# equinor/gordo-components

Hardware: NVIDIA H100
Metric: anomaly windows/sec (64-tag feedforward_hourglass AE, 1k machines x 10k rows per GPU, fused predict+score) (higher is better)
Workload: dtype split tf32/bf16/fp16

## Files before the change

gordo_components_b200/csrc/ffae_infer_tc.cu:

```cuda
#include <atomic>
#include <cuda_bf16.h>
#include <cuda_fp16.h>
#include "gb_common.cuh"
#include "gb_sm90.cuh"

namespace {

using namespace gb::sm90;

constexpr int TILE = 64;
constexpr int NWG_MAX = 3;
constexpr int MAXL = 8;
constexpr int W = 64;
constexpr int BOX_COLS = 32;
constexpr int BOX_COLS_X64 = 16;
constexpr int BOX_BYTES = TILE * BOX_COLS * 4;
constexpr int TILE_BYTES = 2 * BOX_BYTES;
__host__ __device__ constexpr int x_tile_bytes(bool x64) { return x64 ? 2 * TILE_BYTES : TILE_BYTES; }
__host__ __device__ constexpr int stage_bytes(bool x64, int nwg) { return (x_tile_bytes(x64) + TILE_BYTES) * nwg; }
constexpr int OBOX_ROWS = 16;
constexpr int OBOX_BYTES = OBOX_ROWS * BOX_COLS * 4;
__host__ __device__ constexpr int restage_batch(int nthreads) { return (W * W + W + nthreads - 1) / nthreads; }
static_assert(restage_batch(128 * NWG_MAX) == 11, "three warpgroups restage a layer in 11 loads per thread");

struct TcArgs {
  CUtensorMap tm_x, tm_y;
  CUtensorMap tm_o[4];
  int T;
  int L;
  int N[MAXL], Np[MAXL], k16[MAXL];
  int img0_ofs[MAXL], img1_ofs[MAXL], img2_ofs[MAXL];
  int bias_ofs[MAXL];
  int pofs[MAXL];
  int K[MAXL];
  int w_bytes;
  int vec_ofs;
  int stage_ofs;
  int n_jobs, tiles_per_job;
  long pstride;
  const float* params;
  const gb_job* jobs;
  const float *y, *scale, *feat_thr, *agg_thr;
  float *o_model, *o_ts, *o_tu, *o_conf, *o_tots, *o_totu, *o_totconf;
  unsigned int* work_ctr;
  const double *x_scale, *x_offset;
  int xab_ofs;
  long n_x_rows;
};

constexpr float TANH_ARG_SCALE = 2.8853900817779268f;
__device__ __forceinline__ float tanh_from_scaled(float t) {
  float e, r;
  asm("ex2.approx.ftz.f32 %0, %1;" : "=f"(e) : "f"(t));
  asm("rcp.approx.ftz.f32 %0, %1;" : "=f"(r) : "f"(e + 1.0f));
// ... 22 lines not shown
#pragma unroll
  for (int ks = 0; ks < 8; ++ks)
    if (ks < 2 * k16) {
      const uint32_t a[4] = {xhi[ks >> 1][4 * (ks & 1) + 0], xhi[ks >> 1][4 * (ks & 1) + 1], xhi[ks >> 1][4 * (ks & 1) + 2], xhi[ks >> 1][4 * (ks & 1) + 3]};
      if (N == 16) wgmma_rs_tf32_n16(d, a, desc_noswizzle(img0 + ks * step, lbo, 128), ks > 0);
      if (N == 32) wgmma_rs_tf32_n32(d, a, desc_noswizzle(img0 + ks * step, lbo, 128), ks > 0);
      if (N == 48) wgmma_rs_tf32_n48(d, a, desc_noswizzle(img0 + ks * step, lbo, 128), ks > 0);
      if (N == 64) wgmma_rs_tf32_n64(d, a, desc_noswizzle(img0 + ks * step, lbo, 128), ks > 0);
    }
#pragma unroll
  for (int ks = 0; ks < 4; ++ks)
    if (ks < k16) {
      if (N == 16) wgmma_rs_bf16_n16(d, alo[ks], desc_noswizzle(img1 + ks * step, lbo, 128), 1);
      if (N == 32) wgmma_rs_bf16_n32(d, alo[ks], desc_noswizzle(img1 + ks * step, lbo, 128), 1);
      if (N == 48) wgmma_rs_bf16_n48(d, alo[ks], desc_noswizzle(img1 + ks * step, lbo, 128), 1);
      if (N == 64) wgmma_rs_bf16_n64(d, alo[ks], desc_noswizzle(img1 + ks * step, lbo, 128), 1);
    }
#pragma unroll
  for (int ks = 0; ks < 4; ++ks)
    if (ks < k16) {
      if (N == 16) wgmma_rs_bf16_n16(d, abf[ks], desc_noswizzle(img2 + ks * step, lbo, 128), 1);
      if (N == 32) wgmma_rs_bf16_n32(d, abf[ks], desc_noswizzle(img2 + ks * step, lbo, 128), 1);
      if (N == 48) wgmma_rs_bf16_n48(d, abf[ks], desc_noswizzle(img2 + ks * step, lbo, 128), 1);
      if (N == 64) wgmma_rs_bf16_n64(d, abf[ks], desc_noswizzle(img2 + ks * step, lbo, 128), 1);
    }
}
template <int N>
__device__ __forceinline__ void mma_f16(float* d, const uint32_t* a, uint64_t desc, uint32_t acc) {
  if (N == 16) wgmma_rs_f16_n16(d, a, desc, acc);
  if (N == 32) wgmma_rs_f16_n32(d, a, desc, acc);
  if (N == 48) wgmma_rs_f16_n48(d, a, desc, acc);
  if (N == 64) wgmma_rs_f16_n64(d, a, desc, acc);
}
template <int N>
__device__ __forceinline__ void mma_hidden(float* d, const uint32_t (&a1)[4][4], const uint32_t (&a2)[4][4], uint32_t img0, uint32_t img1, int k16) {
  const uint32_t lbo = N * 16, step = 2 * N * 16;
#pragma unroll
  for (int ks = 0; ks < 4; ++ks)
    if (ks < k16) mma_f16<N>(d, a2[ks], desc_noswizzle(img0 + ks * step, lbo, 128), ks > 0);
#pragma unroll
  for (int ks = 0; ks < 4; ++ks)
    if (ks < k16) mma_f16<N>(d, a1[ks], desc_noswizzle(img1 + ks * step, lbo, 128), 1);
#pragma unroll
  for (int ks = 0; ks < 4; ++ks)
    if (ks < k16) mma_f16<N>(d, a1[ks], desc_noswizzle(img0 + ks * step, lbo, 128), 1);
}

__device__ __forceinline__ int box_ofs(int r, int col) { return r * 128 + (((col >> 2) ^ (r & 7)) << 4) + ((col & 3) << 2); }
__device__ __forceinline__ int tile_ofs(int r, int col) { return (col >> 5) * BOX_BYTES + box_ofs(r, col & 31); }
__device__ __forceinline__ int tile_ofs_x64(int r, int col) { return (col >> 4) * BOX_BYTES + r * 128 + ((((col & 15) >> 1) ^ (r & 7)) << 4); }

__device__ __forceinline__ void warpgroup_sync(int wg) { asm volatile("bar.sync %0, 128;" ::"r"(wg + 1) : "memory"); }

__device__ __forceinline__ void fence_acc(float (&d)[32]) {
#pragma unroll
  for (int i = 0; i < 32; ++i) fence_reg(d[i]);
}
template <int R, int C>
__device__ __forceinline__ void fence_frag(uint32_t (&f)[R][C]) {
#pragma unroll
  for (int i = 0; i < R; ++i)
#pragma unroll
    for (int j = 0; j < C; ++j) fence_reg(f[i][j]);
}

template <bool X64, int NWG>
__global__ void __launch_bounds__(128 * NWG, 1) ffae_tc_kernel(const __grid_constant__ TcArgs a) {
  constexpr int NTHREADS = 128 * NWG;
  constexpr int RESTAGE_BATCH = restage_batch(NTHREADS);
  extern __shared__ __align__(1024) uint8_t smem[];
  const int tid = threadIdx.x, lane = tid & 31;
  const int warp = __shfl_sync(0xffffffffu, tid >> 5, 0);
  const int wg = warp >> 2, wq = warp & 3;
  const int g = lane >> 2, t = lane & 3;
  const uint32_t sbase = smem_u32(smem);
  const int TP = a.T, L = a.L;
  const bool has_y = a.y != nullptr;
  const bool totals = has_y && (a.o_tots || a.o_totu || a.o_totconf);
  const float inv_w = 1.0f / (float)TP;

  __shared__ __align__(8) unsigned long long s_bar[2 * NWG];
  const uint32_t stage = (sbase + a.stage_ofs + 1023) & ~1023u;
  const uint32_t xbuf = stage + wg * (x_tile_bytes(X64) + TILE_BYTES), ybuf = xbuf + x_tile_bytes(X64);
  const uint8_t* xs = smem + (xbuf - sbase);
  const uint8_t* ys = smem + (ybuf - sbase);
  const uint32_t bar_x = smem_u32(&s_bar[wg]), bar_y = smem_u32(&s_bar[NWG + wg]);
  const bool leader = (tid & 127) == 0;
  uint32_t x_phase = 0, y_phase = 0;
  const uint32_t obox0 = ybuf + wq * OBOX_BYTES, obox1 = obox0 + BOX_BYTES;
  if (tid == 0) {
    for (int i = 0; i < 2 * NWG; ++i) mbar_init(smem_u32(&s_bar[i]), 1);
    asm volatile("fence.mbarrier_init.release.cluster;" ::: "memory");
  }

  __shared__ int s_item[3];
  __shared__ int s_range[2];
  if (tid == 0) s_range[0] = s_range[1] = 0;
  int cur_slot = -1;

  while (true) {
    if (tid == 0) {
      const int tpj = a.tiles_per_job, g_total = a.n_jobs * tpj;
      int gg = s_range[0], g_end = s_range[1];
      if (gg >= g_end) {
        const int seen = (int)*reinterpret_cast<volatile unsigned int*>(a.work_ctr);
        const int left = g_total - seen, per_cta = left / (int)gridDim.x;
        int size = per_cta * 2 >= 3 * tpj ? tpj : (per_cta >= tpj / 3 ? (tpj + 2) / 3 : (tpj + 5) / 6);
        if (size < 1) size = 1;
        if (seen % tpj != 0 && size > tpj - seen % tpj) size = tpj - seen % tpj;
        gg = (int)atomicAdd(a.work_ctr, (unsigned int)size);
        g_end = gg + size < g_total ? gg + size : g_total;
      }
      if (gg >= g_total) {
        s_item[0] = -1;
      } else {
        const int job_id = gg / tpj, tile_begin = gg - job_id * tpj;
        const int tile_end = min(tpj, tile_begin + (g_end - gg));
        s_item[0] = job_id; s_item[1] = tile_begin; s_item[2] = tile_end;
        gg += tile_end - tile_begin;
      }
      s_range[0] = gg; s_range[1] = g_end;
    }
    __syncthreads();
    const int job_id = s_item[0], tile_begin = s_item[1], tile_end = s_item[2];
    if (job_id < 0) break;
    const gb_job job = a.jobs[job_id];
    const int row_begin = tile_begin * TILE;
    if (row_begin >= job.n_rows) {
      __syncthreads();
      continue;
    }
    const int row_end = min(job.n_rows, tile_end * TILE);
    const int n_tiles = (row_end - row_begin + TILE - 1) / TILE;

    auto load_tile = [&](const CUtensorMap* m, uint32_t buf, uint32_t bar, int tt) {
      const int row = (int)(job.x_row + row_begin + tt * TILE);
      mbar_expect_tx(bar, TILE_BYTES);
      tma_load_2d(buf, m, 0, row, bar);
      tma_load_2d(buf + BOX_BYTES, m, BOX_COLS, row, bar);
    };
    auto load_x64 = [&](int tt) {
      const int row = (int)(job.x_row + row_begin + tt * TILE);
      mbar_expect_tx(bar_x, x_tile_bytes(true));
#pragma unroll
      for (int h = 0; h < 4; ++h) tma_load_2d(xbuf + h * BOX_BYTES, &a.tm_x, BOX_COLS_X64 * h, row, bar_x);
    };
    if (leader && wg < n_tiles) {
      if constexpr (X64) load_x64(wg);
      else load_tile(&a.tm_x, xbuf, bar_x, wg);
    }

    if (job.slot != cur_slot) {
      cur_slot = job.slot;
      const float* P = a.params + (long)job.slot * a.pstride;
      float v[RESTAGE_BATCH], vn[RESTAGE_BATCH];
      auto fetch = [&](float (&dst)[RESTAGE_BATCH], int l) {
        const float* Ws = P + a.pofs[l];
        const int n_l = a.K[l] * a.N[l] + a.N[l];
#pragma unroll
        for (int u = 0; u < RESTAGE_BATCH; ++u) {
          const int i = tid + u * NTHREADS;
          dst[u] = i < n_l ? __ldg(Ws + i) : 0.f;
        }
      };
      fetch(v, 0);
      const bool vt = tid < TP;
      const float sc = vt && a.scale ? __ldg(a.scale + (long)job.slot * TP + tid) : 0.f;
      const float ft = vt && a.feat_thr ? __ldg(a.feat_thr + (long)job.slot * TP + tid) : 0.f;
      for (int i = tid; i < a.w_bytes / 16; i += NTHREADS) reinterpret_cast<uint4*>(smem)[i] = make_uint4(0, 0, 0, 0);
      __syncthreads();
      for (int l = 0; l < L; ++l) {
        if (l + 1 < L) fetch(vn, l + 1);
        const int K = a.K[l], N = a.N[l], Np = a.Np[l], KN = K * N;
        const float bscale = (l + 1 < L) ? TANH_ARG_SCALE : 1.0f;
#pragma unroll
        for (int u = 0; u < RESTAGE_BATCH; ++u) {
          const int i = tid + u * NTHREADS;
          if (i >= KN + N) break;
          if (i >= KN) {
            reinterpret_cast<float*>(smem + a.bias_ofs[l])[i - KN] = v[u] * bscale;
            continue;
          }
          const int k = i / N, n = i - k * N;
          const float w = v[u];
          const int i8 = ((k >> 3) * Np + n) * 8 + (k & 7);
          if (l == 0) {
            const float hi = __uint_as_float((__float_as_uint(w) + 0x1000u) & 0xffffe000u);
            const int kt = tf32_row(k);
            reinterpret_cast<float*>(smem + a.img0_ofs[0])[((kt >> 2) * Np + n) * 4 + (kt & 3)] = hi;
            reinterpret_cast<__nv_bfloat16*>(smem + a.img1_ofs[0])[i8] = __float2bfloat16_rn(hi);
            reinterpret_cast<__nv_bfloat16*>(smem + a.img2_ofs[0])[i8] = __float2bfloat16_rn(w - hi);
          } else {
            const __half w1 = __float2half_rn(w);
            reinterpret_cast<__half*>(smem + a.img0_ofs[l])[i8] = w1;
            reinterpret_cast<__half*>(smem + a.img1_ofs[l])[i8] = __float2half_rn(w - __half2float(w1));
          }
        }
#pragma unroll
        for (int u = 0; u < RESTAGE_BATCH; ++u) v[u] = vn[u];
      }
      float* vec = reinterpret_cast<float*>(smem + a.vec_ofs);
      if (tid < W) {
        vec[tid] = sc;
        vec[W + tid] = vt && a.feat_thr ? 1.0f / ft : 0.f;
      }
      if constexpr (X64) {
        double* xab = reinterpret_cast<double*>(smem + a.xab_ofs);
        if (tid < W) {
          xab[tid] = vt ? __ldg(a.x_scale + (long)job.slot * TP + tid) : 0.0;
          xab[W + tid] = vt ? __ldg(a.x_offset + (long)job.slot * TP + tid) : 0.0;
        }
      }
      fence_proxy_async();
    }
    __syncthreads();

    const float* vec = reinterpret_cast<const float*>(smem + a.vec_ofs);
    for (int tt = wg; tt < n_tiles; tt += NWG) {
      float d[32];
      uint32_t a1[4][4] = {}, a2[4][4] = {};
      {
        float xr[2][16];
        mbar_wait(bar_x, x_phase);
        x_phase ^= 1;
        if constexpr (X64) {
          const double* xab = reinterpret_cast<const double*>(smem + a.xab_ofs);
          const long row0 = job.x_row + row_begin + tt * TILE + wq * 16 + g;
#pragma unroll
          for (int hr = 0; hr < 2; ++hr) {
            const bool live = row0 + 8 * hr < a.n_x_rows;
#pragma unroll
            for (int c = 0; c < 8; ++c) {
              const int col = 8 * c + 2 * t;
              const double2 v = *reinterpret_cast<const double2*>(xs + tile_ofs_x64(wq * 16 + g + 8 * hr, col));
              const double2 s = *reinterpret_cast<const double2*>(xab + col), o = *reinterpret_cast<const double2*>(xab + W + col);
              xr[hr][2 * c] = live ? (float)__dadd_rn(__dmul_rn(v.x, s.x), o.x) : 0.f;
              xr[hr][2 * c + 1] = live ? (float)__dadd_rn(__dmul_rn(v.y, s.y), o.y) : 0.f;
            }
          }
        } else {
#pragma unroll
          for (int hr = 0; hr < 2; ++hr)
#pragma unroll
            for (int c = 0; c < 8; ++c) {
              const float2 v = *reinterpret_cast<const float2*>(xs + tile_ofs(wq * 16 + g + 8 * hr, 8 * c + 2 * t));
              xr[hr][2 * c] = v.x;
              xr[hr][2 * c + 1] = v.y;
            }
        }
        if (lane == 0) bulk_wait_read<0>();
        warpgroup_sync(wg);
        if (leader) {
          if (tt + NWG < n_tiles) {
            if constexpr (X64) load_x64(tt + NWG);
            else load_tile(&a.tm_x, xbuf, bar_x, tt + NWG);
          }
          if (has_y) load_tile(&a.tm_y, ybuf, bar_y, tt);
        }
        uint32_t xhi[4][8], alo[4][4], abf[4][4];
#pragma unroll
        for (int kk = 0; kk < 4; ++kk) {
#pragma unroll
          for (int hh = 0; hh < 2; ++hh) {
            xhi[kk][4 * hh + 0] = __float_as_uint(trunc_tf32(xr[0][4 * kk + 2 * hh]));
            xhi[kk][4 * hh + 1] = __float_as_uint(trunc_tf32(xr[1][4 * kk + 2 * hh]));
            xhi[kk][4 * hh + 2] = __float_as_uint(trunc_tf32(xr[0][4 * kk + 2 * hh + 1]));
            xhi[kk][4 * hh + 3] = __float_as_uint(trunc_tf32(xr[1][4 * kk + 2 * hh + 1]));
          }
#pragma unroll
          for (int q = 0; q < 4; ++q) {
            const float v0 = xr[q & 1][4 * kk + 2 * (q >> 1)], v1 = xr[q & 1][4 * kk + 2 * (q >> 1) + 1];
            alo[kk][q] = pack_bf16(v0 - trunc_tf32(v0), v1 - trunc_tf32(v1));
            abf[kk][q] = pack_bf16(v0, v1);
          }
        }
        const int k16 = a.k16[0];
        const uint32_t i0 = sbase + a.img0_ofs[0], i1 = sbase + a.img1_ofs[0], i2 = sbase + a.img2_ofs[0];
        wgmma_fence();
        switch (a.Np[0]) {
          case 16: mma_layer0<16>(d, xhi, alo, abf, i0, i1, i2, k16); break;
          case 32: mma_layer0<32>(d, xhi, alo, abf, i0, i1, i2, k16); break;
          case 48: mma_layer0<48>(d, xhi, alo, abf, i0, i1, i2, k16); break;
          default: mma_layer0<64>(d, xhi, alo, abf, i0, i1, i2, k16); break;
        }
        wgmma_commit();
        wgmma_wait<0>();
        fence_acc(d);
        fence_frag(xhi);
        fence_frag(alo);
        fence_frag(abf);
      }

      for (int l = 0; l < L; ++l) {
        if (l > 0) {
          const uint32_t i0 = sbase + a.img0_ofs[l], i1 = sbase + a.img1_ofs[l];
          const int k16 = a.k16[l];
          wgmma_fence();
          switch (a.Np[l]) {
            case 16: mma_hidden<16>(d, a1, a2, i0, i1, k16); break;
            case 32: mma_hidden<32>(d, a1, a2, i0, i1, k16); break;
            case 48: mma_hidden<48>(d, a1, a2, i0, i1, k16); break;
            default: mma_hidden<64>(d, a1, a2, i0, i1, k16); break;
          }
          wgmma_commit();
          wgmma_wait<0>();
          fence_acc(d);
          fence_frag(a1);
          fence_frag(a2);
        }
        if (l + 1 == L) break;
        const float* bl = reinterpret_cast<const float*>(smem + a.bias_ofs[l]);
        const int nt = a.Np[l] >> 3;
#pragma unroll
        for (int j = 0; j < 8; ++j) {
          if (j < nt) {
            const float2 b = *reinterpret_cast<const float2*>(bl + 8 * j + 2 * t);
            const float v0 = tanh_from_scaled(fmaf(d[4 * j], TANH_ARG_SCALE, b.x)), v1 = tanh_from_scaled(fmaf(d[4 * j + 1], TANH_ARG_SCALE, b.y));
            const float v2 = tanh_from_scaled(fmaf(d[4 * j + 2], TANH_ARG_SCALE, b.x)), v3 = tanh_from_scaled(fmaf(d[4 * j + 3], TANH_ARG_SCALE, b.y));
            split_f16(v0, v1, a1[j >> 1][2 * (j & 1)], a2[j >> 1][2 * (j & 1)]);
            split_f16(v2, v3, a1[j >> 1][2 * (j & 1) + 1], a2[j >> 1][2 * (j & 1) + 1]);
          }
        }
      }

      const float* bo = reinterpret_cast<const float*>(smem + a.bias_ofs[L - 1]);
      const int wrow = row_begin + tt * TILE + wq * 16;
      const int trow = wrow + g;
      const int nt = a.Np[L - 1] >> 3;
      float2 yr[2][8];
      if (has_y) {
        mbar_wait(bar_y, y_phase);
        y_phase ^= 1;
#pragma unroll
        for (int hr = 0; hr < 2; ++hr)
#pragma unroll
          for (int j = 0; j < 8; ++j) yr[hr][j] = *reinterpret_cast<const float2*>(ys + tile_ofs(wq * 16 + g + 8 * hr, 8 * j + 2 * t));
      }
      auto model_out = [&](int hr, int j) {
        const float2 b = *reinterpret_cast<const float2*>(bo + 8 * j + 2 * t);
        return j < nt ? make_float2(d[4 * j + 2 * hr] + b.x, d[4 * j + 2 * hr + 1] + b.y) : make_float2(0.f, 0.f);
      };

      const int n_live = min(row_end - wrow, OBOX_ROWS);
      const bool want_su = has_y && a.o_totu, want_ss = has_y && (a.o_tots || a.o_totconf);
      float ss[2] = {0.f, 0.f}, su[2] = {0.f, 0.f};
      if (n_live > 0) {
        const int nh = TP > BOX_COLS ? 2 : 1;
        int k = 0;
#pragma unroll
        for (int arr = 0; arr < 4; ++arr) {
          if (arr == 1 && has_y) {
#pragma unroll
            for (int hr = 0; hr < 2; ++hr)
#pragma unroll
              for (int j = 0; j < 8; ++j) {
                const float2 m = model_out(hr, j);
                yr[hr][j] = make_float2(fabsf(m.x - yr[hr][j].x), fabsf(m.y - yr[hr][j].y));
              }
          }
          float* o = arr == 0 ? a.o_model : arr == 1 ? a.o_tu : arr == 2 ? a.o_ts : a.o_conf;
          const bool put = o != nullptr && (arr == 0 || has_y);
          const bool acc = arr == 1 ? want_su : arr == 2 ? want_ss : false;
          if (!put && !acc) continue;
          const float* sv = vec + (arr == 3 ? W : 0);
          const uint32_t box0 = nh == 2 || (k & 1) == 0 ? obox0 : obox1;
          if (put) {
            if (lane == 0) {
              if (nh == 2 && k >= 1) bulk_wait_read<0>();
              if (nh == 1 && k >= 2) bulk_wait_read<1>();
            }
            __syncwarp();
          }
#pragma unroll
          for (int h = 0; h < 2; ++h) {
            if (h == nh) break;
            uint8_t* bs = smem + ((h ? obox1 : box0) - sbase);
#pragma unroll
            for (int hr = 0; hr < 2; ++hr)
#pragma unroll
              for (int jj = 0; jj < 4; ++jj) {
                const int j = 4 * h + jj, col = 8 * j + 2 * t;
                float2 v = arr == 0 ? model_out(hr, j) : yr[hr][j];
                if (arr > 1) {
                  const float2 s = *reinterpret_cast<const float2*>(sv + col);
                  v = make_float2(v.x * s.x, v.y * s.y);
                }
                if (acc && col < TP) {
                  const float q = __fmaf_rn(v.x, v.x, __fmul_rn(v.y, v.y));
                  if (arr == 1) su[hr] = __fadd_rn(su[hr], q);
                  else ss[hr] = __fadd_rn(ss[hr], q);
                }
                if (put) *reinterpret_cast<float2*>(bs + box_ofs(g + 8 * hr, 8 * jj + 2 * t)) = v;
              }
          }
          if (!put) continue;
          fence_proxy_async();
          __syncwarp();
          if (n_live == OBOX_ROWS) {
            if (lane == 0) {
              for (int h = 0; h < nh; ++h) tma_store_2d(&a.tm_o[arr], h ? obox1 : box0, BOX_COLS * h, (int)(job.out_row + wrow));
              bulk_commit();
            }
          } else {
            for (int h = 0; h < nh; ++h) {
              const uint8_t* bs = smem + ((h ? obox1 : box0) - sbase);
              const int cols = min(BOX_COLS, TP - BOX_COLS * h);
              for (int i = lane; i < n_live * 8; i += 32) {
                const int r = i >> 3, c = i & 7;
                if (4 * c < cols)
                  __stcs(reinterpret_cast<float4*>(o + (job.out_row + wrow + r) * (long)TP + BOX_COLS * h + 4 * c),
                         *reinterpret_cast<const float4*>(bs + box_ofs(r, 4 * c)));
              }
            }
          }
          ++k;
        }
      }
      if (totals) {
#pragma unroll
        for (int hr = 0; hr < 2; ++hr) {
          ss[hr] += __shfl_xor_sync(0xffffffffu, ss[hr], 1);
          ss[hr] += __shfl_xor_sync(0xffffffffu, ss[hr], 2);
          su[hr] += __shfl_xor_sync(0xffffffffu, su[hr], 1);
          su[hr] += __shfl_xor_sync(0xffffffffu, su[hr], 2);
          const int r = trow + 8 * hr;
          if (t == 0 && r < row_end) {
            const long go = job.out_row + r;
            const float ts_ = ss[hr] * inv_w, tu_ = su[hr] * inv_w;
            if (a.o_tots) a.o_tots[go] = ts_;
            if (a.o_totu) a.o_totu[go] = tu_;
            if (a.o_totconf) a.o_totconf[go] = ts_ / __ldg(a.agg_thr + job.slot);
          }
        }
      }
    }
    __syncthreads();
  }
  if (lane == 0) bulk_wait<0>();
}

constexpr int WORK_CTRS = 1024;
__device__ unsigned int g_work_ctr[WORK_CTRS];

int plan_smem(const gb_ffnet* net, TcArgs& a, bool x64 = false, int nwg = NWG_MAX) {
  const int L = net->n_layers;
  a.L = L;
  a.T = net->dims[0];
  int ofs = 0, pofs = 0;
  for (int l = 0; l < L; ++l) {
    a.K[l] = net->dims[l];
    a.N[l] = net->dims[l + 1];
    a.Np[l] = gb::round_up(a.N[l], 16);
    a.k16[l] = gb::round_up(a.K[l], 16) / 16;
    a.pofs[l] = pofs;
    pofs += a.K[l] * a.N[l] + a.N[l];
    const int kp = a.k16[l] * 16;
    a.img0_ofs[l] = ofs;
    ofs += kp * a.Np[l] * (l == 0 ? 4 : 2);
    a.img1_ofs[l] = ofs;
    ofs += kp * a.Np[l] * 2;
    if (l == 0) {
      a.img2_ofs[l] = ofs;
      ofs += kp * a.Np[l] * 2;
    }
  }
  for (int l = 0; l < L; ++l) {
    a.bias_ofs[l] = ofs;
    ofs += W * 4;
  }
// ... 54 lines not shown
  GB_REQUIRE(nwg > 0, GB_E_SMEM, "tensor-core variant with float64 x: the weights and two warpgroups' x / y tiles of this stack need %d "
             "bytes of shared memory (227 KB per SM)", smem);
  return nwg;
}

extern "C" int gb_ffae_infer_score_tc(const gb_ffnet* net, const float* params, const gb_job* jobs, int32_t n_jobs, int32_t max_rows,
                                      int64_t n_x_rows, int64_t n_out_rows, const void* x, const double* x_scale, const double* x_offset,
                                      const float* y, const float* scale, const float* feat_thr, const float* agg_thr, float* out_model,
                                      float* out_tag_scaled, float* out_tag_unscaled, float* out_total_scaled, float* out_total_unscaled,
                                      float* out_conf, float* out_total_conf, int32_t flags, void* stream) {
  int rc = gb_ffae_tc_supported(net);
  if (rc != GB_OK) return rc;
  GB_REQUIRE(flags == 0, GB_E_ARG, "variant bits above the low byte must be 0");
  GB_REQUIRE(n_x_rows > 0 && n_out_rows > 0, GB_E_ARG, "the tensor-core variant needs the row counts of x and of the outputs");
  const bool x64 = x_scale != nullptr;
  TcArgs a{};
  int nwg = NWG_MAX, smem_i = 0;
  if (x64) {
    nwg = gb_ffae_tc_warpgroups_x64(net);
    if (nwg < 0) return nwg;
    x64_warpgroups(net, a, &smem_i);
  } else {
    smem_i = plan_smem(net, a);
  }
  const size_t smem = (size_t)smem_i;
  GB_REQUIRE(n_x_rows < (1L << 31), GB_E_ARG, "%ld rows of x: TMA row coordinates are 32-bit", (long)n_x_rows);
  GB_REQUIRE(n_out_rows < (1L << 31), GB_E_ARG, "%ld output rows: TMA row coordinates are 32-bit", (long)n_out_rows);
  {
    CUresult r = x64 ? gb::sm90::encode_map_2d(&a.tm_x, CU_TENSOR_MAP_DATA_TYPE_FLOAT64, 8, x, n_x_rows, a.T, BOX_COLS_X64, TILE)
                     : gb::sm90::encode_map_2d(&a.tm_x, CU_TENSOR_MAP_DATA_TYPE_FLOAT32, 4, x, n_x_rows, a.T, BOX_COLS, TILE);
    if (r == CUDA_SUCCESS && y) r = gb::sm90::encode_map_2d(&a.tm_y, CU_TENSOR_MAP_DATA_TYPE_FLOAT32, 4, y, n_x_rows, a.T, BOX_COLS, TILE);
    float* const outs[4] = {out_model, out_tag_unscaled, out_tag_scaled, out_conf};
    for (int i = 0; i < 4; ++i)
      if (r == CUDA_SUCCESS && outs[i]) r = gb::sm90::encode_map_2d(&a.tm_o[i], CU_TENSOR_MAP_DATA_TYPE_FLOAT32, 4, outs[i], n_out_rows, a.T, BOX_COLS, OBOX_ROWS);
    GB_REQUIRE(r != CUDA_ERROR_NOT_FOUND, GB_E_CUDA, "cuTensorMapEncodeTiled is not available from the driver");
    GB_REQUIRE(r == CUDA_SUCCESS, GB_E_CUDA, "cuTensorMapEncodeTiled (x / y / outputs) failed with CUresult %d", (int)r);
  }

  int dev = 0, sms = 132;
  GB_CUDA_CHECK(cudaGetDevice(&dev));
  GB_CUDA_CHECK(cudaDeviceGetAttribute(&sms, cudaDevAttrMultiProcessorCount, dev));
  const int tiles_per_job = (max_rows + TILE - 1) / TILE;
  a.tiles_per_job = tiles_per_job;
  a.n_jobs = n_jobs;
  a.pstride = (long)gb_ffnet_param_stride(net);
  a.params = params; a.jobs = jobs; a.y = y; a.scale = scale; a.feat_thr = feat_thr; a.agg_thr = agg_thr;
  a.o_model = out_model; a.o_ts = out_tag_scaled; a.o_tu = out_tag_unscaled; a.o_conf = out_conf;
  a.o_tots = out_total_scaled; a.o_totu = out_total_unscaled; a.o_totconf = out_total_conf;
  a.x_scale = x_scale; a.x_offset = x_offset; a.n_x_rows = (long)n_x_rows;

  const long g_total = (long)n_jobs * tiles_per_job;
  GB_REQUIRE(g_total < (1L << 31), GB_E_ARG, "%ld tiles in one launch: split the fleet", g_total);
  const int grid = (int)(g_total < sms ? g_total : sms);
  {
    static std::atomic<unsigned> next_ctr{0};
    void* base = nullptr;
    GB_CUDA_CHECK(cudaGetSymbolAddress(&base, g_work_ctr));
    a.work_ctr = static_cast<unsigned int*>(base) + (next_ctr.fetch_add(1) % WORK_CTRS);
    GB_CUDA_CHECK(cudaMemsetAsync(a.work_ctr, 0, sizeof(unsigned int), (cudaStream_t)stream));
  }
  auto launch = [&](auto kern, int nthreads) -> int {
    GB_CUDA_CHECK(cudaFuncSetAttribute(kern, cudaFuncAttributeMaxDynamicSharedMemorySize, (int)smem));
    kern<<<grid, nthreads, smem, (cudaStream_t)stream>>>(a);
    return GB_OK;
  };
  rc = !x64 ? launch(ffae_tc_kernel<false, 3>, 384) : nwg == 3 ? launch(ffae_tc_kernel<true, 3>, 384) : launch(ffae_tc_kernel<true, 2>, 256);
  if (rc != GB_OK) return rc;
// ... 4 lines not shown
```

gordo_components_b200/csrc/gb_sm90.cuh:

```cuda
#pragma once
#include <cuda.h>
#include <stdint.h>

namespace gb {
namespace sm90 {

__device__ __forceinline__ uint32_t smem_u32(const void* p) { return (uint32_t)__cvta_generic_to_shared(p); }

__device__ __forceinline__ uint64_t desc_noswizzle(uint32_t smem_addr, uint32_t lbo, uint32_t sbo) {
  return (uint64_t)((smem_addr >> 4) & 0x3FFF) | ((uint64_t)((lbo >> 4) & 0x3FFF) << 16) | ((uint64_t)((sbo >> 4) & 0x3FFF) << 32);
}
__device__ __forceinline__ uint64_t desc_sw128(uint32_t smem_addr) {
  return (uint64_t)((smem_addr >> 4) & 0x3FFF) | ((uint64_t)1 << 16) | ((uint64_t)(1024 >> 4) << 32) | ((uint64_t)1 << 62);
}

__device__ __forceinline__ void wgmma_fence() { asm volatile("wgmma.fence.sync.aligned;" ::: "memory"); }
__device__ __forceinline__ void wgmma_commit() { asm volatile("wgmma.commit_group.sync.aligned;" ::: "memory"); }
template <int N>
__device__ __forceinline__ void wgmma_wait() { asm volatile("wgmma.wait_group.sync.aligned %0;" ::"n"(N) : "memory"); }
__device__ __forceinline__ void fence_reg(float& r) { asm volatile("" : "+f"(r)::"memory"); }
__device__ __forceinline__ void fence_reg(uint32_t& r) { asm volatile("" : "+r"(r)::"memory"); }

__device__ __forceinline__ void fence_proxy_async() { asm volatile("fence.proxy.async.shared::cta;" ::: "memory"); }

__device__ __forceinline__ void mbar_init(uint32_t bar, uint32_t count) { asm volatile("mbarrier.init.shared::cta.b64 [%0], %1;" ::"r"(bar), "r"(count)); }
__device__ __forceinline__ void mbar_expect_tx(uint32_t bar, uint32_t bytes) {
  asm volatile("mbarrier.arrive.expect_tx.shared::cta.b64 _, [%0], %1;" ::"r"(bar), "r"(bytes) : "memory");
}
__device__ __forceinline__ void mbar_arrive(uint32_t bar) { asm volatile("mbarrier.arrive.shared::cta.b64 _, [%0];" ::"r"(bar) : "memory"); }
__device__ __forceinline__ void mbar_wait(uint32_t bar, uint32_t parity) {
  asm volatile(
      "{\n\t"
      ".reg .pred p;\n\t"
      "WAIT_%=:\n\t"
      "mbarrier.try_wait.parity.shared::cta.b64 p, [%0], %1;\n\t"
      "@p bra DONE_%=;\n\t"
      "bra WAIT_%=;\n\t"
      "DONE_%=:\n\t"
      "}" ::"r"(bar), "r"(parity)
      : "memory");
}
__device__ __forceinline__ void tma_load_2d(uint32_t dst, const CUtensorMap* map, int c0, int c1, uint32_t bar) {
  asm volatile("cp.async.bulk.tensor.2d.shared::cluster.global.mbarrier::complete_tx::bytes [%0], [%1, {%2, %3}], [%4];" ::"r"(dst), "l"(map),
               "r"(c0), "r"(c1), "r"(bar)
               : "memory");
}
__device__ __forceinline__ void tma_store_2d(const CUtensorMap* map, uint32_t src, int c0, int c1) {
  asm volatile("cp.async.bulk.tensor.2d.global.shared::cta.bulk_group [%0, {%2, %3}], [%1];" ::"l"(map), "r"(src), "r"(c0), "r"(c1) : "memory");
}
__device__ __forceinline__ void bulk_commit() { asm volatile("cp.async.bulk.commit_group;" ::: "memory"); }
template <int N>
__device__ __forceinline__ void bulk_wait_read() { asm volatile("cp.async.bulk.wait_group.read %0;" ::"n"(N) : "memory"); }
template <int N>
__device__ __forceinline__ void bulk_wait() { asm volatile("cp.async.bulk.wait_group %0;" ::"n"(N) : "memory"); }

inline CUresult encode_map_2d(CUtensorMap* map, CUtensorMapDataType type, int elem_bytes, const void* base, long rows, long cols, int box_cols,
                              int box_rows) {
  typedef CUresult (*EncodeTiledFn)(CUtensorMap*, CUtensorMapDataType, cuuint32_t, void*, const cuuint64_t*, const cuuint64_t*, const cuuint32_t*,
                                    const cuuint32_t*, CUtensorMapInterleave, CUtensorMapSwizzle, CUtensorMapL2promotion, CUtensorMapFloatOOBfill);
  static EncodeTiledFn fn = nullptr;
  if (!fn) {
    void* p = nullptr;
    cudaDriverEntryPointQueryResult q;
    if (cudaGetDriverEntryPoint("cuTensorMapEncodeTiled", &p, cudaEnableDefault, &q) != cudaSuccess || q != cudaDriverEntryPointSuccess)
      return CUDA_ERROR_NOT_FOUND;
    fn = reinterpret_cast<EncodeTiledFn>(p);
  }
  const cuuint64_t dims[2] = {(cuuint64_t)cols, (cuuint64_t)rows};
  const cuuint64_t strides[1] = {(cuuint64_t)cols * elem_bytes};
  const cuuint32_t box[2] = {(cuuint32_t)box_cols, (cuuint32_t)box_rows};
  const cuuint32_t estr[2] = {1, 1};
  return fn(map, type, 2, const_cast<void*>(base), dims, strides, box, estr, CU_TENSOR_MAP_INTERLEAVE_NONE, CU_TENSOR_MAP_SWIZZLE_128B,
            CU_TENSOR_MAP_L2_PROMOTION_L2_128B, CU_TENSOR_MAP_FLOAT_OOB_FILL_NONE);
}

__device__ __forceinline__ void wgmma_rs_f16_n16(float* d, const uint32_t* a, uint64_t bdesc, uint32_t accumulate) {
  asm volatile(
      "{\n.reg .pred p;\nsetp.ne.b32 p, %13, 0;\n"
      "wgmma.mma_async.sync.aligned.m64n16k16.f32.f16.f16 {%0, %1, %2, %3, %4, %5, %6, %7}, {%8, %9, %10, %11}, %12, p, 1, 1, 0;\n}\n"
      : "+f"(d[0]), "+f"(d[1]), "+f"(d[2]), "+f"(d[3]), "+f"(d[4]), "+f"(d[5]), "+f"(d[6]), "+f"(d[7])
      : "r"(a[0]), "r"(a[1]), "r"(a[2]), "r"(a[3]), "l"(bdesc), "r"(accumulate));
}
__device__ __forceinline__ void wgmma_rs_f16_n32(float* d, const uint32_t* a, uint64_t bdesc, uint32_t accumulate) {
  asm volatile(
      "{\n.reg .pred p;\nsetp.ne.b32 p, %21, 0;\n"
      "wgmma.mma_async.sync.aligned.m64n32k16.f32.f16.f16 {%0, %1, %2, %3, %4, %5, %6, %7, %8, %9, %10, %11, %12, %13, %14, %15}, {%16, %17, %18, %19}, %20, p, 1, 1, 0;\n}\n"
      : "+f"(d[0]), "+f"(d[1]), "+f"(d[2]), "+f"(d[3]), "+f"(d[4]), "+f"(d[5]), "+f"(d[6]), "+f"(d[7]), "+f"(d[8]), "+f"(d[9]), "+f"(d[10]), "+f"(d[11]), "+f"(d[12]), "+f"(d[13]), "+f"(d[14]), "+f"(d[15])
      : "r"(a[0]), "r"(a[1]), "r"(a[2]), "r"(a[3]), "l"(bdesc), "r"(accumulate));
}
__device__ __forceinline__ void wgmma_rs_f16_n48(float* d, const uint32_t* a, uint64_t bdesc, uint32_t accumulate) {
  asm volatile(
      "{\n.reg .pred p;\nsetp.ne.b32 p, %29, 0;\n"
      "wgmma.mma_async.sync.aligned.m64n48k16.f32.f16.f16 {%0, %1, %2, %3, %4, %5, %6, %7, %8, %9, %10, %11, %12, %13, %14, %15, %16, %17, %18, %19, %20, %21, %22, %23}, {%24, %25, %26, %27}, %28, p, 1, 1, 0;\n}\n"
      : "+f"(d[0]), "+f"(d[1]), "+f"(d[2]), "+f"(d[3]), "+f"(d[4]), "+f"(d[5]), "+f"(d[6]), "+f"(d[7]), "+f"(d[8]), "+f"(d[9]), "+f"(d[10]), "+f"(d[11]), "+f"(d[12]), "+f"(d[13]), "+f"(d[14]), "+f"(d[15]), "+f"(d[16]), "+f"(d[17]), "+f"(d[18]), "+f"(d[19]), "+f"(d[20]), "+f"(d[21]), "+f"(d[22]), "+f"(d[23])
      : "r"(a[0]), "r"(a[1]), "r"(a[2]), "r"(a[3]), "l"(bdesc), "r"(accumulate));
}
__device__ __forceinline__ void wgmma_rs_f16_n64(float* d, const uint32_t* a, uint64_t bdesc, uint32_t accumulate) {
  asm volatile(
      "{\n.reg .pred p;\nsetp.ne.b32 p, %37, 0;\n"
      "wgmma.mma_async.sync.aligned.m64n64k16.f32.f16.f16 {%0, %1, %2, %3, %4, %5, %6, %7, %8, %9, %10, %11, %12, %13, %14, %15, %16, %17, %18, %19, %20, %21, %22, %23, %24, %25, %26, %27, %28, %29, %30, %31}, {%32, %33, %34, %35}, %36, p, 1, 1, 0;\n}\n"
      : "+f"(d[0]), "+f"(d[1]), "+f"(d[2]), "+f"(d[3]), "+f"(d[4]), "+f"(d[5]), "+f"(d[6]), "+f"(d[7]), "+f"(d[8]), "+f"(d[9]), "+f"(d[10]), "+f"(d[11]), "+f"(d[12]), "+f"(d[13]), "+f"(d[14]), "+f"(d[15]), "+f"(d[16]), "+f"(d[17]), "+f"(d[18]), "+f"(d[19]), "+f"(d[20]), "+f"(d[21]), "+f"(d[22]), "+f"(d[23]), "+f"(d[24]), "+f"(d[25]), "+f"(d[26]), "+f"(d[27]), "+f"(d[28]), "+f"(d[29]), "+f"(d[30]), "+f"(d[31])
      : "r"(a[0]), "r"(a[1]), "r"(a[2]), "r"(a[3]), "l"(bdesc), "r"(accumulate));
}
__device__ __forceinline__ void wgmma_rs_bf16_n16(float* d, const uint32_t* a, uint64_t bdesc, uint32_t accumulate) {
  asm volatile(
      "{\n.reg .pred p;\nsetp.ne.b32 p, %13, 0;\n"
// ... 64 lines not shown
```

Measured before the change: 1.714 billion.

## Prefetch next work item, its first x tiles and its weights during current item

Work claiming is moved to a dedicated thread in the last warpgroup and double-buffered, so the next item (job descriptor included) is claimed while the current one finishes, and an mbarrier publishes it. Once an item completes, each warpgroup issues the TMA load of its first x tile for the next item, and all threads prefetch the first PF layers of the next slot's weights and per-tag vectors into registers before the block barrier. The per-slot smem zeroing now happens only on the first restage. This targets the serialized claim, load and restage latency between items, at the cost of many more live registers (PF x RESTAGE_BATCH floats) and a more complex control flow.

After: 1.733 billion (median of 6 runs). +1.1%, better.

```diff
diff --git a/gordo_components_b200/csrc/ffae_infer_tc.cu b/gordo_components_b200/csrc/ffae_infer_tc.cu
--- a/gordo_components_b200/csrc/ffae_infer_tc.cu
+++ b/gordo_components_b200/csrc/ffae_infer_tc.cu
@@ -144,6 +144,7 @@
 __global__ void __launch_bounds__(128 * NWG, 1) ffae_tc_kernel(const __grid_constant__ TcArgs a) {
   constexpr int NTHREADS = 128 * NWG;
   constexpr int RESTAGE_BATCH = restage_batch(NTHREADS);
+  constexpr int PF = NWG == 3 ? 2 : 6;
   extern __shared__ __align__(1024) uint8_t smem[];
   const int tid = threadIdx.x, lane = tid & 31;
   const int warp = __shfl_sync(0xffffffffu, tid >> 5, 0);
@@ -155,98 +156,129 @@
   const bool totals = has_y && (a.o_tots || a.o_totu || a.o_totconf);
   const float inv_w = 1.0f / (float)TP;
 
-  __shared__ __align__(8) unsigned long long s_bar[2 * NWG];
+  __shared__ __align__(8) unsigned long long s_bar[2 * NWG + 1];
   const uint32_t stage = (sbase + a.stage_ofs + 1023) & ~1023u;
   const uint32_t xbuf = stage + wg * (x_tile_bytes(X64) + TILE_BYTES), ybuf = xbuf + x_tile_bytes(X64);
   const uint8_t* xs = smem + (xbuf - sbase);
   const uint8_t* ys = smem + (ybuf - sbase);
-  const uint32_t bar_x = smem_u32(&s_bar[wg]), bar_y = smem_u32(&s_bar[NWG + wg]);
+  const uint32_t bar_x = smem_u32(&s_bar[wg]), bar_y = smem_u32(&s_bar[NWG + wg]), bar_claim = smem_u32(&s_bar[2 * NWG]);
   const bool leader = (tid & 127) == 0;
-  uint32_t x_phase = 0, y_phase = 0;
+  uint32_t x_phase = 0, y_phase = 0, claim_phase = 0;
   const uint32_t obox0 = ybuf + wq * OBOX_BYTES, obox1 = obox0 + BOX_BYTES;
   if (tid == 0) {
-    for (int i = 0; i < 2 * NWG; ++i) mbar_init(smem_u32(&s_bar[i]), 1);
+    for (int i = 0; i < 2 * NWG + 1; ++i) mbar_init(smem_u32(&s_bar[i]), 1);
     asm volatile("fence.mbarrier_init.release.cluster;" ::: "memory");
   }
 
-  __shared__ int s_item[3];
+  auto load_tile = [&](const CUtensorMap* m, uint32_t buf, uint32_t bar, long row) {
+    mbar_expect_tx(bar, TILE_BYTES);
+    tma_load_2d(buf, m, 0, (int)row, bar);
+    tma_load_2d(buf + BOX_BYTES, m, BOX_COLS, (int)row, bar);
+  };
+  auto load_x = [&](long row) {
+    if constexpr (X64) {
+      mbar_expect_tx(bar_x, x_tile_bytes(true));
+#pragma unroll
+      for (int h = 0; h < 4; ++h) tma_load_2d(xbuf + h * BOX_BYTES, &a.tm_x, BOX_COLS_X64 * h, (int)row, bar_x);
+    } else {
+      load_tile(&a.tm_x, xbuf, bar_x, row);
+    }
+  };
+
+  constexpr int CLAIMER = 128 * (NWG - 1);
+  __shared__ int s_item[2][3];
+  __shared__ gb_job s_job[2];
   __shared__ int s_range[2];
-  if (tid == 0) s_range[0] = s_range[1] = 0;
+  auto claim = [&](int b) {
+    int* item = s_item[b];
+    const int tpj = a.tiles_per_job, g_total = a.n_jobs * tpj;
+    int gg = s_range[0], g_end = s_range[1];
+    if (gg >= g_end) {
+      const int seen = (int)*reinterpret_cast<volatile unsigned int*>(a.work_ctr);
+      const int left = g_total - seen, per_cta = left / (int)gridDim.x;
+      int size = per_cta * 2 >= 3 * tpj ? tpj : (per_cta >= tpj / 3 ? (tpj + 2) / 3 : (tpj + 5) / 6);
+      if (size < 1) size = 1;
+      if (seen % tpj != 0 && size > tpj - seen % tpj) size = tpj - seen % tpj;
+      gg = (int)atomicAdd(a.work_ctr, (unsigned int)size);
+      g_end = gg + size < g_total ? gg + size : g_total;
+    }
+    if (gg >= g_total) {
+      item[0] = -1;
+    } else {
+      const int job_id = gg / tpj, tile_begin = gg - job_id * tpj;
+      const int tile_end = min(tpj, tile_begin + (g_end - gg));
+      item[0] = job_id; item[1] = tile_begin; item[2] = tile_end;
+      s_job[b] = a.jobs[job_id];
+      gg += tile_end - tile_begin;
+    }
+    s_range[0] = gg; s_range[1] = g_end;
+  };
+  if (tid == CLAIMER) {
+    s_range[0] = s_range[1] = 0;
+    claim(0);
+  }
+  __syncthreads();
+  int cur = 0;
   int cur_slot = -1;
+  bool x_early = false;
+
+  float pv[PF][RESTAGE_BATCH];
+  float pv_sc, pv_ft;
+  double pv_xs, pv_xo;
+  int pv_slot = -1;
+  auto fetch_layer = [&](float (&dst)[RESTAGE_BATCH], const float* P, int l) {
+    const bool live = l < L;
+    const float* Ws = P + (live ? a.pofs[l] : 0);
+    const int n_l = live ? a.K[l] * a.N[l] + a.N[l] : 0;
+#pragma unroll
+    for (int u = 0; u < RESTAGE_BATCH; ++u) {
+      const int i = tid + u * NTHREADS;
+      dst[u] = i < n_l ? __ldg(Ws + i) : 0.f;
+    }
+  };
+  auto fetch = [&](int slot, bool on) {
+    const float* P = a.params + (long)max(slot, 0) * a.pstride;
+#pragma unroll
+    for (int l = 0; l < PF; ++l) fetch_layer(pv[l], P, on ? l : MAXL);
+    const bool vt = on && tid < TP;
+    pv_sc = vt && a.scale ? __ldg(a.scale + (long)slot * TP + tid) : 0.f;
+    pv_ft = vt && a.feat_thr ? __ldg(a.feat_thr + (long)slot * TP + tid) : 0.f;
+    if constexpr (X64) {
+      pv_xs = vt ? __ldg(a.x_scale + (long)slot * TP + tid) : 0.0;
+      pv_xo = vt ? __ldg(a.x_offset + (long)slot * TP + tid) : 0.0;
+    }
+    pv_slot = on ? slot : -1;
+  };
+  fetch(-1, false);
 
   while (true) {
-    if (tid == 0) {
-      const int tpj = a.tiles_per_job, g_total = a.n_jobs * tpj;
-      int gg = s_range[0], g_end = s_range[1];
-      if (gg >= g_end) {
-        const int seen = (int)*reinterpret_cast<volatile unsigned int*>(a.work_ctr);
-        const int left = g_total - seen, per_cta = left / (int)gridDim.x;
-        int size = per_cta * 2 >= 3 * tpj ? tpj : (per_cta >= tpj / 3 ? (tpj + 2) / 3 : (tpj + 5) / 6);
-        if (size < 1) size = 1;
-        if (seen % tpj != 0 && size > tpj - seen % tpj) size = tpj - seen % tpj;
-        gg = (int)atomicAdd(a.work_ctr, (unsigned int)size);
-        g_end = gg + size < g_total ? gg + size : g_total;
-      }
-      if (gg >= g_total) {
-        s_item[0] = -1;
-      } else {
-        const int job_id = gg / tpj, tile_begin = gg - job_id * tpj;
-        const int tile_end = min(tpj, tile_begin + (g_end - gg));
-        s_item[0] = job_id; s_item[1] = tile_begin; s_item[2] = tile_end;
-        gg += tile_end - tile_begin;
-      }
-      s_range[0] = gg; s_range[1] = g_end;
-    }
-    __syncthreads();
-    const int job_id = s_item[0], tile_begin = s_item[1], tile_end = s_item[2];
+    const int job_id = s_item[cur][0], tile_begin = s_item[cur][1], tile_end = s_item[cur][2];
     if (job_id < 0) break;
-    const gb_job job = a.jobs[job_id];
+    const gb_job job = s_job[cur];
     const int row_begin = tile_begin * TILE;
     if (row_begin >= job.n_rows) {
+      if (tid == CLAIMER) claim(cur ^ 1);
       __syncthreads();
+      cur ^= 1;
+      x_early = false;
       continue;
     }
     const int row_end = min(job.n_rows, tile_end * TILE);
     const int n_tiles = (row_end - row_begin + TILE - 1) / TILE;
 
-    auto load_tile = [&](const CUtensorMap* m, uint32_t buf, uint32_t bar, int tt) {
-      const int row = (int)(job.x_row + row_begin + tt * TILE);
-      mbar_expect_tx(bar, TILE_BYTES);
-      tma_load_2d(buf, m, 0, row, bar);
-      tma_load_2d(buf + BOX_BYTES, m, BOX_COLS, row, bar);
-    };
-    auto load_x64 = [&](int tt) {
-      const int row = (int)(job.x_row + row_begin + tt * TILE);
-      mbar_expect_tx(bar_x, x_tile_bytes(true));
-#pragma unroll
-      for (int h = 0; h < 4; ++h) tma_load_2d(xbuf + h * BOX_BYTES, &a.tm_x, BOX_COLS_X64 * h, row, bar_x);
-    };
-    if (leader && wg < n_tiles) {
-      if constexpr (X64) load_x64(wg);
-      else load_tile(&a.tm_x, xbuf, bar_x, wg);
-    }
+    if (leader && wg < n_tiles && !x_early) load_x(job.x_row + row_begin + wg * TILE);
 
     if (job.slot != cur_slot) {
+      if (pv_slot != job.slot) fetch(job.slot, true);
+      if (cur_slot < 0) {
+        for (int i = tid; i < a.w_bytes / 16; i += NTHREADS) reinterpret_cast<uint4*>(smem)[i] = make_uint4(0, 0, 0, 0);
+        __syncthreads();
+      }
       cur_slot = job.slot;
       const float* P = a.params + (long)job.slot * a.pstride;
-      float v[RESTAGE_BATCH], vn[RESTAGE_BATCH];
-      auto fetch = [&](float (&dst)[RESTAGE_BATCH], int l) {
-        const float* Ws = P + a.pofs[l];
-        const int n_l = a.K[l] * a.N[l] + a.N[l];
-#pragma unroll
-        for (int u = 0; u < RESTAGE_BATCH; ++u) {
-          const int i = tid + u * NTHREADS;
-          dst[u] = i < n_l ? __ldg(Ws + i) : 0.f;
-        }
-      };
-      fetch(v, 0);
-      const bool vt = tid < TP;
-      const float sc = vt && a.scale ? __ldg(a.scale + (long)job.slot * TP + tid) : 0.f;
-      const float ft = vt && a.feat_thr ? __ldg(a.feat_thr + (long)job.slot * TP + tid) : 0.f;
-      for (int i = tid; i < a.w_bytes / 16; i += NTHREADS) reinterpret_cast<uint4*>(smem)[i] = make_uint4(0, 0, 0, 0);
-      __syncthreads();
       for (int l = 0; l < L; ++l) {
-        if (l + 1 < L) fetch(vn, l + 1);
+        float vn[RESTAGE_BATCH];
+        fetch_layer(vn, P, l + PF);
         const int K = a.K[l], N = a.N[l], Np = a.Np[l], KN = K * N;
         const float bscale = (l + 1 < L) ? TANH_ARG_SCALE : 1.0f;
 #pragma unroll
@@ -254,11 +286,11 @@
           const int i = tid + u * NTHREADS;
           if (i >= KN + N) break;
           if (i >= KN) {
-            reinterpret_cast<float*>(smem + a.bias_ofs[l])[i - KN] = v[u] * bscale;
+            reinterpret_cast<float*>(smem + a.bias_ofs[l])[i - KN] = pv[0][u] * bscale;
             continue;
           }
           const int k = i / N, n = i - k * N;
-          const float w = v[u];
+          const float w = pv[0][u];
           const int i8 = ((k >> 3) * Np + n) * 8 + (k & 7);
           if (l == 0) {
             const float hi = __uint_as_float((__float_as_uint(w) + 0x1000u) & 0xffffe000u);
@@ -273,18 +305,22 @@
           }
         }
 #pragma unroll
-        for (int u = 0; u < RESTAGE_BATCH; ++u) v[u] = vn[u];
+        for (int u = 0; u < RESTAGE_BATCH; ++u) {
+#pragma unroll
+          for (int m = 0; m + 1 < PF; ++m) pv[m][u] = pv[m + 1][u];
+          pv[PF - 1][u] = vn[u];
+        }
       }
       float* vec = reinterpret_cast<float*>(smem + a.vec_ofs);
       if (tid < W) {
-        vec[tid] = sc;
-        vec[W + tid] = vt && a.feat_thr ? 1.0f / ft : 0.f;
+        vec[tid] = pv_sc;
+        vec[W + tid] = tid < TP && a.feat_thr ? 1.0f / pv_ft : 0.f;
       }
       if constexpr (X64) {
         double* xab = reinterpret_cast<double*>(smem + a.xab_ofs);
         if (tid < W) {
-          xab[tid] = vt ? __ldg(a.x_scale + (long)job.slot * TP + tid) : 0.0;
-          xab[W + tid] = vt ? __ldg(a.x_offset + (long)job.slot * TP + tid) : 0.0;
+          xab[tid] = pv_xs;
+          xab[W + tid] = pv_xo;
         }
       }
       fence_proxy_async();
@@ -327,11 +363,9 @@
         if (lane == 0) bulk_wait_read<0>();
         warpgroup_sync(wg);
         if (leader) {
-          if (tt + NWG < n_tiles) {
-            if constexpr (X64) load_x64(tt + NWG);
-            else load_tile(&a.tm_x, xbuf, bar_x, tt + NWG);
-          }
-          if (has_y) load_tile(&a.tm_y, ybuf, bar_y, tt);
+          const long row = job.x_row + row_begin + tt * TILE;
+          if (tt + NWG < n_tiles) load_x(row + NWG * TILE);
+          if (has_y) load_tile(&a.tm_y, ybuf, bar_y, row);
         }
         uint32_t xhi[4][8], alo[4][4], abf[4][4];
 #pragma unroll
@@ -510,7 +544,30 @@
         }
       }
     }
+
+    if (tid == CLAIMER) {
+      claim(cur ^ 1);
+      mbar_arrive(bar_claim);
+    }
+    mbar_wait(bar_claim, claim_phase);
+    claim_phase ^= 1;
+    bool restage_next = false;
+    int next_slot = -1;
+    x_early = false;
+    if (s_item[cur ^ 1][0] >= 0) {
+      const gb_job nx = s_job[cur ^ 1];
+      const int nrb = s_item[cur ^ 1][1] * TILE;
+      if (nrb < nx.n_rows) {
+        const int n_next = (min(nx.n_rows, s_item[cur ^ 1][2] * TILE) - nrb + TILE - 1) / TILE;
+        x_early = wg < n_next;
+        if (leader && x_early) load_x(nx.x_row + nrb + wg * TILE);
+        restage_next = nx.slot != cur_slot;
+        next_slot = nx.slot;
+      }
+    }
+    fetch(next_slot, restage_next);
     __syncthreads();
+    cur ^= 1;
   }
   if (lane == 0) bulk_wait<0>();
 }
```

## Store full 64-col output rows via 3D TMA boxes and specialize hidden-layer K loop

Applied to the files above, without the earlier changes.

When the tag count equals 64, output tiles are written through a 3D tensor map that covers both 32-column halves of 8 rows at once. Each TMA store therefore writes whole contiguous output rows instead of two half-row column boxes. The shared-memory staging layout is remapped to match, including the partial-tile fallback. Separately, the hidden-layer wgmma loop gets a compile-time K16 count when three warpgroups are used, and the wgmma fence moves inside the helper. The remapped staging offsets add address-arithmetic complexity and a risk of layout mistakes.

Result: faster. 1.697 billion before, 1.723 billion after (median of 6 runs) (+1.5%).

```diff
diff --git a/gordo_components_b200/csrc/ffae_infer_tc.cu b/gordo_components_b200/csrc/ffae_infer_tc.cu
--- a/gordo_components_b200/csrc/ffae_infer_tc.cu
+++ b/gordo_components_b200/csrc/ffae_infer_tc.cu
@@ -20,6 +20,7 @@
 __host__ __device__ constexpr int stage_bytes(bool x64, int nwg) { return (x_tile_bytes(x64) + TILE_BYTES) * nwg; }
 constexpr int OBOX_ROWS = 16;
 constexpr int OBOX_BYTES = OBOX_ROWS * BOX_COLS * 4;
+constexpr int WBOX_ROWS = 8;
 __host__ __device__ constexpr int restage_batch(int nthreads) { return (W * W + W + nthreads - 1) / nthreads; }
 static_assert(restage_batch(128 * NWG_MAX) == 11, "three warpgroups restage a layer in 11 loads per thread");
 
@@ -108,18 +109,33 @@
   if (N == 48) wgmma_rs_f16_n48(d, a, desc, acc);
   if (N == 64) wgmma_rs_f16_n64(d, a, desc, acc);
 }
-template <int N>
+template <int N, int K16>
 __device__ __forceinline__ void mma_hidden(float* d, const uint32_t (&a1)[4][4], const uint32_t (&a2)[4][4], uint32_t img0, uint32_t img1, int k16) {
   const uint32_t lbo = N * 16, step = 2 * N * 16;
+  const int nk = K16 ? K16 : k16;
+  wgmma_fence();
 #pragma unroll
   for (int ks = 0; ks < 4; ++ks)
-    if (ks < k16) mma_f16<N>(d, a2[ks], desc_noswizzle(img0 + ks * step, lbo, 128), ks > 0);
+    if (ks < nk) mma_f16<N>(d, a2[ks], desc_noswizzle(img0 + ks * step, lbo, 128), ks > 0);
 #pragma unroll
   for (int ks = 0; ks < 4; ++ks)
-    if (ks < k16) mma_f16<N>(d, a1[ks], desc_noswizzle(img1 + ks * step, lbo, 128), 1);
+    if (ks < nk) mma_f16<N>(d, a1[ks], desc_noswizzle(img1 + ks * step, lbo, 128), 1);
 #pragma unroll
   for (int ks = 0; ks < 4; ++ks)
-    if (ks < k16) mma_f16<N>(d, a1[ks], desc_noswizzle(img0 + ks * step, lbo, 128), 1);
+    if (ks < nk) mma_f16<N>(d, a1[ks], desc_noswizzle(img0 + ks * step, lbo, 128), 1);
+}
+template <int N, bool FIXED_K>
+__device__ __forceinline__ void mma_hidden_k(float* d, const uint32_t (&a1)[4][4], const uint32_t (&a2)[4][4], uint32_t img0, uint32_t img1, int k16) {
+  if constexpr (!FIXED_K) {
+    mma_hidden<N, 0>(d, a1, a2, img0, img1, k16);
+  } else {
+    switch (k16) {
+      case 1: mma_hidden<N, 1>(d, a1, a2, img0, img1, k16); break;
+      case 2: mma_hidden<N, 2>(d, a1, a2, img0, img1, k16); break;
+      case 3: mma_hidden<N, 3>(d, a1, a2, img0, img1, k16); break;
+      default: mma_hidden<N, 4>(d, a1, a2, img0, img1, k16); break;
+    }
+  }
 }
 
 __device__ __forceinline__ int box_ofs(int r, int col) { return r * 128 + (((col >> 2) ^ (r & 7)) << 4) + ((col & 3) << 2); }
@@ -371,12 +387,11 @@
         if (l > 0) {
           const uint32_t i0 = sbase + a.img0_ofs[l], i1 = sbase + a.img1_ofs[l];
           const int k16 = a.k16[l];
-          wgmma_fence();
           switch (a.Np[l]) {
-            case 16: mma_hidden<16>(d, a1, a2, i0, i1, k16); break;
-            case 32: mma_hidden<32>(d, a1, a2, i0, i1, k16); break;
-            case 48: mma_hidden<48>(d, a1, a2, i0, i1, k16); break;
-            default: mma_hidden<64>(d, a1, a2, i0, i1, k16); break;
+            case 16: mma_hidden_k<16, NWG == 3>(d, a1, a2, i0, i1, k16); break;
+            case 32: mma_hidden_k<32, NWG == 3>(d, a1, a2, i0, i1, k16); break;
+            case 48: mma_hidden_k<48, NWG == 3>(d, a1, a2, i0, i1, k16); break;
+            default: mma_hidden_k<64, NWG == 3>(d, a1, a2, i0, i1, k16); break;
           }
           wgmma_commit();
           wgmma_wait<0>();
@@ -417,6 +432,8 @@
         return j < nt ? make_float2(d[4 * j + 2 * hr] + b.x, d[4 * j + 2 * hr + 1] + b.y) : make_float2(0.f, 0.f);
       };
 
+      const bool whole_row = TP == W;
+      const int box_swap = whole_row ? 1024 : BOX_BYTES;
       const int n_live = min(row_end - wrow, OBOX_ROWS);
       const bool want_su = has_y && a.o_totu, want_ss = has_y && (a.o_tots || a.o_totconf);
       float ss[2] = {0.f, 0.f}, su[2] = {0.f, 0.f};
@@ -450,9 +467,9 @@
 #pragma unroll
           for (int h = 0; h < 2; ++h) {
             if (h == nh) break;
-            uint8_t* bs = smem + ((h ? obox1 : box0) - sbase);
-#pragma unroll
-            for (int hr = 0; hr < 2; ++hr)
+#pragma unroll
+            for (int hr = 0; hr < 2; ++hr) {
+              uint8_t* bs = smem + (box0 - sbase) + (h == hr ? h * (BOX_BYTES + 1024) : h ? box_swap : BOX_BYTES + 1024 - box_swap);
 #pragma unroll
               for (int jj = 0; jj < 4; ++jj) {
                 const int j = 4 * h + jj, col = 8 * j + 2 * t;
@@ -466,26 +483,32 @@
                   if (arr == 1) su[hr] = __fadd_rn(su[hr], q);
                   else ss[hr] = __fadd_rn(ss[hr], q);
                 }
-                if (put) *reinterpret_cast<float2*>(bs + box_ofs(g + 8 * hr, 8 * jj + 2 * t)) = v;
+                if (put) *reinterpret_cast<float2*>(bs + box_ofs(g, 8 * jj + 2 * t)) = v;
               }
+            }
           }
           if (!put) continue;
           fence_proxy_async();
           __syncwarp();
           if (n_live == OBOX_ROWS) {
             if (lane == 0) {
-              for (int h = 0; h < nh; ++h) tma_store_2d(&a.tm_o[arr], h ? obox1 : box0, BOX_COLS * h, (int)(job.out_row + wrow));
+              if (whole_row) {
+                tma_store_3d(&a.tm_o[arr], obox0, 0, (int)(job.out_row + wrow), 0);
+                tma_store_3d(&a.tm_o[arr], obox1, 0, (int)(job.out_row + wrow + WBOX_ROWS), 0);
+              } else {
+                for (int h = 0; h < nh; ++h) tma_store_2d(&a.tm_o[arr], h ? obox1 : box0, BOX_COLS * h, (int)(job.out_row + wrow));
+              }
               bulk_commit();
             }
           } else {
             for (int h = 0; h < nh; ++h) {
-              const uint8_t* bs = smem + ((h ? obox1 : box0) - sbase);
               const int cols = min(BOX_COLS, TP - BOX_COLS * h);
               for (int i = lane; i < n_live * 8; i += 32) {
                 const int r = i >> 3, c = i & 7;
+                const int bo = whole_row ? (r >> 3) * BOX_BYTES + h * 1024 : h * BOX_BYTES + (r >> 3) * 1024;
                 if (4 * c < cols)
                   __stcs(reinterpret_cast<float4*>(o + (job.out_row + wrow + r) * (long)TP + BOX_COLS * h + 4 * c),
-                         *reinterpret_cast<const float4*>(bs + box_ofs(r, 4 * c)));
+                         *reinterpret_cast<const float4*>(smem + (box0 - sbase) + bo + box_ofs(r & 7, 4 * c)));
               }
             }
           }
@@ -631,7 +654,9 @@
     if (r == CUDA_SUCCESS && y) r = gb::sm90::encode_map_2d(&a.tm_y, CU_TENSOR_MAP_DATA_TYPE_FLOAT32, 4, y, n_x_rows, a.T, BOX_COLS, TILE);
     float* const outs[4] = {out_model, out_tag_unscaled, out_tag_scaled, out_conf};
     for (int i = 0; i < 4; ++i)
-      if (r == CUDA_SUCCESS && outs[i]) r = gb::sm90::encode_map_2d(&a.tm_o[i], CU_TENSOR_MAP_DATA_TYPE_FLOAT32, 4, outs[i], n_out_rows, a.T, BOX_COLS, OBOX_ROWS);
+      if (r == CUDA_SUCCESS && outs[i])
+        r = a.T == W ? gb::sm90::encode_map_row_halves(&a.tm_o[i], outs[i], n_out_rows, WBOX_ROWS)
+                     : gb::sm90::encode_map_2d(&a.tm_o[i], CU_TENSOR_MAP_DATA_TYPE_FLOAT32, 4, outs[i], n_out_rows, a.T, BOX_COLS, OBOX_ROWS);
     GB_REQUIRE(r != CUDA_ERROR_NOT_FOUND, GB_E_CUDA, "cuTensorMapEncodeTiled is not available from the driver");
     GB_REQUIRE(r == CUDA_SUCCESS, GB_E_CUDA, "cuTensorMapEncodeTiled (x / y / outputs) failed with CUresult %d", (int)r);
   }
diff --git a/gordo_components_b200/csrc/gb_sm90.cuh b/gordo_components_b200/csrc/gb_sm90.cuh
--- a/gordo_components_b200/csrc/gb_sm90.cuh
+++ b/gordo_components_b200/csrc/gb_sm90.cuh
@@ -48,30 +48,51 @@
 __device__ __forceinline__ void tma_store_2d(const CUtensorMap* map, uint32_t src, int c0, int c1) {
   asm volatile("cp.async.bulk.tensor.2d.global.shared::cta.bulk_group [%0, {%2, %3}], [%1];" ::"l"(map), "r"(src), "r"(c0), "r"(c1) : "memory");
 }
+__device__ __forceinline__ void tma_store_3d(const CUtensorMap* map, uint32_t src, int c0, int c1, int c2) {
+  asm volatile("cp.async.bulk.tensor.3d.global.shared::cta.bulk_group [%0, {%2, %3, %4}], [%1];" ::"l"(map), "r"(src), "r"(c0), "r"(c1), "r"(c2)
+               : "memory");
+}
 __device__ __forceinline__ void bulk_commit() { asm volatile("cp.async.bulk.commit_group;" ::: "memory"); }
 template <int N>
 __device__ __forceinline__ void bulk_wait_read() { asm volatile("cp.async.bulk.wait_group.read %0;" ::"n"(N) : "memory"); }
 template <int N>
 __device__ __forceinline__ void bulk_wait() { asm volatile("cp.async.bulk.wait_group %0;" ::"n"(N) : "memory"); }
 
-inline CUresult encode_map_2d(CUtensorMap* map, CUtensorMapDataType type, int elem_bytes, const void* base, long rows, long cols, int box_cols,
-                              int box_rows) {
-  typedef CUresult (*EncodeTiledFn)(CUtensorMap*, CUtensorMapDataType, cuuint32_t, void*, const cuuint64_t*, const cuuint64_t*, const cuuint32_t*,
-                                    const cuuint32_t*, CUtensorMapInterleave, CUtensorMapSwizzle, CUtensorMapL2promotion, CUtensorMapFloatOOBfill);
+typedef CUresult (*EncodeTiledFn)(CUtensorMap*, CUtensorMapDataType, cuuint32_t, void*, const cuuint64_t*, const cuuint64_t*, const cuuint32_t*,
+                                  const cuuint32_t*, CUtensorMapInterleave, CUtensorMapSwizzle, CUtensorMapL2promotion, CUtensorMapFloatOOBfill);
+inline EncodeTiledFn encode_tiled_fn() {
   static EncodeTiledFn fn = nullptr;
   if (!fn) {
     void* p = nullptr;
     cudaDriverEntryPointQueryResult q;
     if (cudaGetDriverEntryPoint("cuTensorMapEncodeTiled", &p, cudaEnableDefault, &q) != cudaSuccess || q != cudaDriverEntryPointSuccess)
-      return CUDA_ERROR_NOT_FOUND;
+      return nullptr;
     fn = reinterpret_cast<EncodeTiledFn>(p);
   }
+  return fn;
+}
+
+inline CUresult encode_map_2d(CUtensorMap* map, CUtensorMapDataType type, int elem_bytes, const void* base, long rows, long cols, int box_cols,
+                              int box_rows) {
+  const EncodeTiledFn fn = encode_tiled_fn();
+  if (!fn) return CUDA_ERROR_NOT_FOUND;
   const cuuint64_t dims[2] = {(cuuint64_t)cols, (cuuint64_t)rows};
   const cuuint64_t strides[1] = {(cuuint64_t)cols * elem_bytes};
   const cuuint32_t box[2] = {(cuuint32_t)box_cols, (cuuint32_t)box_rows};
   const cuuint32_t estr[2] = {1, 1};
   return fn(map, type, 2, const_cast<void*>(base), dims, strides, box, estr, CU_TENSOR_MAP_INTERLEAVE_NONE, CU_TENSOR_MAP_SWIZZLE_128B,
             CU_TENSOR_MAP_L2_PROMOTION_L2_128B, CU_TENSOR_MAP_FLOAT_OOB_FILL_NONE);
+}
+
+inline CUresult encode_map_row_halves(CUtensorMap* map, const void* base, long rows, int box_rows) {
+  const EncodeTiledFn fn = encode_tiled_fn();
+  if (!fn) return CUDA_ERROR_NOT_FOUND;
+  const cuuint64_t dims[3] = {32, (cuuint64_t)rows, 2};
+  const cuuint64_t strides[2] = {64 * 4, 32 * 4};
+  const cuuint32_t box[3] = {32, (cuuint32_t)box_rows, 2};
+  const cuuint32_t estr[3] = {1, 1, 1};
+  return fn(map, CU_TENSOR_MAP_DATA_TYPE_FLOAT32, 3, const_cast<void*>(base), dims, strides, box, estr, CU_TENSOR_MAP_INTERLEAVE_NONE,
+            CU_TENSOR_MAP_SWIZZLE_128B, CU_TENSOR_MAP_L2_PROMOTION_L2_128B, CU_TENSOR_MAP_FLOAT_OOB_FILL_NONE);
 }
 
 __device__ __forceinline__ void wgmma_rs_f16_n16(float* d, const uint32_t* a, uint64_t bdesc, uint32_t accumulate) {
```
